# rhymes-ai/Aria

Hardware: NVIDIA H100
Metric: Aria-25.3B bf16 prefill tokens/sec (higher is better)
Workload: dtype bf16

## Files before the change

aria_b200/_lib.py:

```python
from __future__ import annotations

import ctypes as C
import os

_HERE = os.path.dirname(os.path.abspath(__file__))
LIB_PATH = os.environ.get("ARIA_B200_LIB") or os.path.join(_HERE, "libaria_b200.so")

ARIA_OK = 0
B_NK, B_GKN, B_GNK = 0, 1, 2
EPI_LINEAR, EPI_SWIGLU, EPI_HEADS = 0, 1, 2
ACT_NONE, ACT_GELU_TANH, ACT_GELU_NEW = 0, 1, 2

_ERR = {-1: "bad argument", -2: "unsupported shape", -3: "CUDA error"}

vp = C.c_void_p
i32 = C.c_int32
i64 = C.c_int64
f32 = C.c_float


class GemmDesc(C.Structure):

    _fields_ = [
        ("a", vp), ("lda", i64), ("m", i64), ("n", i64), ("k", i64),
        ("b", vp * 3), ("n_seg", i32), ("b_layout", i32),
        ("num_groups", i32), ("group_offsets", vp), ("group_mod", i32),
        ("epilogue", i32), ("act", i32),
        ("bias", vp * 3), ("residual", vp), ("ldr", i64),
        ("out", vp * 3), ("ldo", i64),
        ("head_dim", i32), ("head_ld", i32), ("rows_per_batch", i32), ("pos0", i32),
        ("stride_b", i64), ("stride_h", i64),
        ("rope_mask", i32), ("rope_cos", vp), ("rope_sin", vp), ("position_ids", vp),
        ("group_counts", vp), ("a_rows", i64), ("out_group_base", vp), ("out_group_row0", vp),
    ]


SIGNATURES = {
    "aria_abi_version": (i32, []),
    "aria_build_arch": (C.c_char_p, []),
    "aria_gemm": (i32, [C.POINTER(GemmDesc), vp]),
    "aria_grouped_gemm": (i32, [vp, vp, vp, vp, i64, i64, i64, i32, vp]),
    "aria_offsets_from_counts": (i32, [vp, vp, i32, vp]),
    "aria_router_topk": (i32, [vp, vp, vp, vp, vp, vp, i64, i32, i32, i32, vp]),
    "aria_route_from_logits": (i32, [vp, vp, vp, vp, i64, i32, i32, vp]),
    "aria_route_given_indices": (i32, [vp, vp, vp, vp, i64, i32, i32, vp]),
    "aria_build_permutation": (i32, [vp, vp, vp, vp, vp, i64, i32, i32, i32, vp]),
    "aria_quantize_fp8_cols": (i32, [vp, vp, vp, i32, i64, i64, vp]),
    "aria_grouped_gemm_fp8": (i32, [vp, vp, vp, vp, vp, i64, i64, i64, i32, i32, vp]),
    "aria_permute_quantize_fp8_rows": (i32, [vp, vp, vp, vp, i64, i32, vp]),
    "aria_grouped_gemm_w8a8": (i32, [vp, vp, vp, vp, vp, vp, i64, i64, i64, i32, i32, vp]),
    "aria_grouped_wgrad": (i32, [vp, i64, vp, i64, vp, vp, i64, i64, i64, i32, i32, vp]),
    "aria_moe_block_fwd_workspace_bytes": (i64, [i64, i32, i32, i32, i32, i32]),
    "aria_moe_block_fwd": (i32, [vp, vp, vp, vp, vp, vp, vp, vp, i64, i32, i32, i32, i32, i32, vp, vp, i64, vp, vp]),
    "aria_moe_block_fwd_fp8": (i32, [vp, vp, vp, vp, vp, vp, vp, vp, vp, vp, i64, i32, i32, i32, i32, i32, vp, vp, i64, vp, vp]),
    "aria_moe_block_fwd_w8a8": (i32, [vp, vp, vp, vp, vp, vp, vp, vp, vp, vp, i64, i32, i32, i32, i32, i32, vp, vp, i64, vp, vp]),
    "aria_swiglu_fwd": (i32, [vp, vp, i64, i32, vp]),
    "aria_swiglu_bwd": (i32, [vp, vp, vp, i64, i32, vp]),
    "aria_combine_bwd": (i32, [vp, vp, vp, vp, vp, vp, i64, i32, i32, vp]),
    "aria_router_bwd": (i32, [vp, vp, vp, vp, i64, i32, i32, vp]),
    "aria_router_aux_workspace_bytes": (C.c_size_t, [i32]),
    "aria_router_aux_loss": (i32, [vp, vp, vp, i64, i32, i32, f32, f32, vp, C.c_size_t, vp]),
    "aria_router_aux_bwd": (i32, [vp, vp, vp, i64, i32, i32, f32, f32, f32, vp]),
    "aria_permute_rows": (i32, [vp, vp, vp, i64, i32, vp]),
# ... 65 lines not shown
```

aria_b200/csrc/gemm.cu:

```cuda
#include <cuda_fp8.h>

#include "gemm_common.cuh"

namespace aria {

constexpr int GEMM_STAGES = 4;
constexpr int FP8_LAND_STAGES = 3;
constexpr int FP8_CONVERT_WARPS = 3;
constexpr int PAIR_MIN_ROWS = 2048;
template <int BN, bool B_FP8 = false>
constexpr int gemm_smem_bytes() {
  return 1024  + GEMM_STAGES * (A_STAGE_BYTES + BN * BK * 2) + BM * acc_ld(BN) * 4 + 256  +
         (B_FP8 ? FP8_LAND_STAGES * BN * BK : 0);
}
static_assert(gemm_smem_bytes<128, true>() <= 232448, "fp8 landing ring must fit the opt-in shared memory of a block");

ARIA_DEVICE void e4m3x16_to_bf16(const uint4 v, uint4& lo, uint4& hi) {
  const uint32_t w[4] = {v.x, v.y, v.z, v.w};
  uint32_t o[8];
#pragma unroll
  for (int i = 0; i < 4; ++i) {
#pragma unroll
    for (int h = 0; h < 2; ++h) {
      const __half2_raw hr = __nv_cvt_fp8x2_to_halfraw2(static_cast<__nv_fp8x2_storage_t>(w[i] >> (16 * h)), __NV_E4M3);
      const float2 f = __half22float2(__half2(hr));
      o[2 * i + h] = pack_bf16(f.x, f.y);
    }
  }
  lo = make_uint4(o[0], o[1], o[2], o[3]);
  hi = make_uint4(o[4], o[5], o[6], o[7]);
}

template <bool PAIR> ARIA_DEVICE int first_tile() { return PAIR ? blockIdx.x >> 1 : blockIdx.x; }
template <bool PAIR> ARIA_DEVICE int tile_step() { return PAIR ? gridDim.x >> 1 : gridDim.x; }
template <bool PAIR> ARIA_DEVICE int pair_sched_n(int n_tiles) { return PAIR ? (n_tiles + 1) / 2 : n_tiles; }

template <int BN, bool B_MN>
ARIA_DEVICE void wgmma_tile_k16(float (&acc)[BN / 2], uint64_t da, uint64_t db) {
  if constexpr (BN == 128) wgmma_m64n128_ss<0, B_MN ? 1 : 0>(acc, da, db, 1u);
  else wgmma_m64n144_ss<0, B_MN ? 1 : 0>(acc, da, db, 1u);
}

template <int BN, bool B_MN, int EPI, bool B_FP8 = false, bool PAIR = false>
__global__ void __launch_bounds__(GEMM_THREADS, 1)
gemm_kernel(const __grid_constant__ CUtensorMap tmA, const __grid_constant__ CUtensorMap tmB0,
            const __grid_constant__ CUtensorMap tmB1, const __grid_constant__ CUtensorMap tmB2, const GemmParams p) {
  constexpr int B_STAGE_BYTES = BN * BK * 2;
  constexpr int STAGE_BYTES = A_STAGE_BYTES + B_STAGE_BYTES;
  constexpr int STAGES = GEMM_STAGES;
  constexpr int ACC_LD = acc_ld(BN);
  constexpr int OUT_BN = (EPI == ARIA_EPI_SWIGLU) ? BN / 2 : BN;
  static_assert(BN == 128 || BN == 144, "tile widths with a wgmma wrapper");
  static_assert(!B_FP8 || (B_MN && BN == 128 && EPI != ARIA_EPI_HEADS), "fp8 B: grouped [G, K, N] weights, 128-wide tiles");
  static_assert(!PAIR || (!B_MN && !B_FP8), "CTA pairs: dense K-major bf16 B");
  constexpr int LAND_BYTES = BN * BK;

  uint8_t* smem = smem_1024();
  float* stg = reinterpret_cast<float*>(smem + STAGES * STAGE_BYTES);
  const BarrierRing<STAGES> bar(stg + BM * ACC_LD);
  const BarrierRing<FP8_LAND_STAGES> land_bar(bar.empty + STAGES);
  uint8_t* land = reinterpret_cast<uint8_t*>(bar.full) + 256;

  const int warp = threadIdx.x >> 5;
  const int lane = threadIdx.x & 31;
  const int wg = threadIdx.x >> 7;

  if (warp == 0 && lane == 0) {
    prefetch_tmap(&tmA);
    prefetch_tmap(&tmB0);
    if (p.n_seg > 1 || EPI == ARIA_EPI_SWIGLU) prefetch_tmap(&tmB1);
    if (p.n_seg > 2) prefetch_tmap(&tmB2);
    bar.init(B_FP8 ? 1 + FP8_CONVERT_WARPS : 1, PAIR ? 2 * CONSUMER_WARPS : CONSUMER_WARPS);
    if constexpr (B_FP8) land_bar.init(1, FP8_CONVERT_WARPS);
    fence_mbar_init();
  }
// ... 324 lines not shown
  d.a = a;
  d.lda = k;
  d.m = rows;
  d.n = n;
  d.k = k;
  d.b[0] = b;
  d.n_seg = 1;
  d.b_layout = ARIA_B_GKN;
  d.num_groups = groups;
  d.group_offsets = offsets;
  d.epilogue = epilogue;
  d.out[0] = out;
  d.ldo = n;
  return d;
}

static int64_t max_tiles(const aria_gemm_desc_t* d, int BN, int64_t groups) {
  const bool swiglu = d->epilogue == ARIA_EPI_SWIGLU;
  const int out_bn = swiglu ? BN / 2 : BN;
  const int64_t n_out_total = d->n * (swiglu ? 1 : d->n_seg);
  return (n_out_total + out_bn - 1) / out_bn * ((d->m + BM - 1) / BM + groups);
}

static int gemm_run(const aria_gemm_desc_t* d, const float* b_scale, cudaStream_t stream) {
  ARIA_CHECK_ARG(d != nullptr);
  ARIA_CHECK_ARG(d->a && d->b[0] && d->out[0]);
  ARIA_CHECK_ARG(d->m >= 0 && d->n > 0 && d->k > 0);
  ARIA_CHECK_ARG(d->n % 8 == 0 && d->k % 8 == 0 && d->lda % 8 == 0);
  ARIA_CHECK_ARG(d->n_seg >= 1 && d->n_seg <= 3);
  ARIA_CHECK_ARG(d->num_groups >= 1 && (d->group_mod >= 0 || d->num_groups % (-d->group_mod) == 0));
  ARIA_CHECK_ARG((reinterpret_cast<uintptr_t>(d->a) & 15) == 0 && (reinterpret_cast<uintptr_t>(d->out[0]) & 15) == 0);
  if (d->m == 0) return ARIA_OK;
  const bool b_mn = d->b_layout == ARIA_B_GKN;
  const bool b_gnk = d->b_layout == ARIA_B_GNK;
  const bool swiglu = d->epilogue == ARIA_EPI_SWIGLU;
  if (b_mn) {
    ARIA_CHECK_ARG(d->n_seg == 1);
    ARIA_CHECK_ARG(d->k % BK == 0 || (d->num_groups == 1 && d->group_mod == 0));
    ARIA_CHECK_ARG(d->n % 64 == 0);
    ARIA_CHECK_ARG(d->epilogue != ARIA_EPI_HEADS);
  } else {
    ARIA_CHECK_ARG(d->num_groups == 1 || d->n_seg == 1);
    if (swiglu) ARIA_CHECK_ARG(d->n_seg == 2 && d->b[1]);
    if (b_gnk) ARIA_CHECK_ARG(d->n_seg == 1 && !swiglu && d->epilogue == ARIA_EPI_LINEAR && d->n % 128 == 0);
    else ARIA_CHECK_ARG(d->num_groups == 1);
  }
  if (d->num_groups > 1) ARIA_CHECK_ARG(d->group_offsets != nullptr);
  if (d->group_counts) ARIA_CHECK_ARG(d->group_offsets != nullptr);
  if (d->out_group_base) ARIA_CHECK_ARG(d->out_group_row0 != nullptr && d->epilogue == ARIA_EPI_LINEAR && d->group_offsets != nullptr);
  ARIA_CHECK_ARG(d->a_rows == 0 || d->a_rows >= d->m);

  int BN = 128;
  if (d->epilogue == ARIA_EPI_HEADS) {
    ARIA_CHECK_ARG(d->head_dim > 0 && d->head_dim % 8 == 0 && d->head_ld >= d->head_dim && d->n % d->head_dim == 0);
    if (d->rope_mask) ARIA_CHECK_ARG(d->head_dim == 128 && d->rope_cos && d->rope_sin);
    if (d->n % 128 != 0) {
      ARIA_CHECK_ARG(!d->rope_mask && d->n % 144 == 0);
      BN = 144;
    }
    for (int s = 0; s < d->n_seg; ++s) ARIA_CHECK_ARG(d->out[s] && d->b[s]);
  } else {
    if (swiglu) ARIA_CHECK_ARG(d->n % 64 == 0);
    if (d->n_seg > 1 && !swiglu) ARIA_CHECK_ARG(d->n % BN == 0);
  }

  const bool pair = !b_scale && d->b_layout == ARIA_B_NK && d->num_groups == 1 && !d->group_offsets &&
                    d->epilogue == ARIA_EPI_LINEAR && d->m >= PAIR_MIN_ROWS;

  CUtensorMap tmA, tmB[3];
  int rc = make_tmap_2d(&tmA, d->a, d->k, d->a_rows > 0 ? d->a_rows : d->m, d->lda * 2, BK, pair ? BM / 2 : BM);
  if (rc) return rc;
  if (b_mn) {
    const uint64_t ncols = swiglu ? 2 * d->n : d->n;
    const uint64_t n_weights = d->group_mod > 0 ? d->group_mod : (d->group_mod < 0 ? d->num_groups / (-d->group_mod) : d->num_groups);
    rc = b_scale ? make_tmap_2d(&tmB[0], d->b[0], ncols, n_weights * d->k, ncols, 64, BK, CU_TENSOR_MAP_SWIZZLE_NONE,
                                CU_TENSOR_MAP_DATA_TYPE_UINT8)
                 : make_tmap_2d(&tmB[0], d->b[0], ncols, n_weights * d->k, ncols * 2, 64, BK);
    if (rc) return rc;
    tmB[1] = tmB[0];
    tmB[2] = tmB[0];
  } else {
    const int nb = swiglu ? 2 : d->n_seg;
    const uint32_t box_rows = swiglu ? BN / 2 : BN;
    for (int s = 0; s < 3; ++s) {
      const void* ptr = s < nb ? d->b[s] : d->b[0];
      const uint64_t b_rows = b_gnk ? static_cast<uint64_t>(d->group_mod > 0 ? d->group_mod : (d->group_mod < 0 ? d->num_groups / (-d->group_mod) : d->num_groups)) * d->n : d->n;
      rc = make_tmap_2d(&tmB[s], ptr, d->k, b_rows, d->k * 2, BK, box_rows);
      if (rc) return rc;
    }
  }

  const GemmParams p = gemm_params(d, b_scale);
  const int64_t tiles = max_tiles(d, BN, d->num_groups > 1 ? d->num_groups : 0);
  if (pair) {
    const int64_t m_tiles = (d->m + BM - 1) / BM, pairs = (tiles / m_tiles + 1) / 2 * m_tiles;
    return launch_persistent_pairs<gemm_kernel<128, false, ARIA_EPI_LINEAR, false, true>>(
        "gemm_kernel", GEMM_THREADS, gemm_smem_bytes<128>(), pairs, stream, tmA, tmB[0], tmB[1], tmB[2], p);
  }
#define ARIA_LAUNCH(BN_, MN_, EPI_, ...)                                                                                     \
  return launch_persistent<gemm_kernel<BN_, MN_, EPI_, ##__VA_ARGS__>>("gemm_kernel", GEMM_THREADS,                          \
                                                                       gemm_smem_bytes<BN_, ##__VA_ARGS__>(), tiles, stream, \
                                                                       tmA, tmB[0], tmB[1], tmB[2], p)
  if (b_scale) {
    if (swiglu) ARIA_LAUNCH(128, true, ARIA_EPI_SWIGLU, true);
    ARIA_LAUNCH(128, true, ARIA_EPI_LINEAR, true);
  }
  if (d->epilogue == ARIA_EPI_HEADS) {
    if (BN == 128) ARIA_LAUNCH(128, false, ARIA_EPI_HEADS);
    ARIA_LAUNCH(144, false, ARIA_EPI_HEADS);
  }
  if (swiglu) {
    if (b_mn) ARIA_LAUNCH(128, true, ARIA_EPI_SWIGLU);
    ARIA_LAUNCH(128, false, ARIA_EPI_SWIGLU);
  }
  if (b_mn) ARIA_LAUNCH(128, true, ARIA_EPI_LINEAR);
  ARIA_LAUNCH(128, false, ARIA_EPI_LINEAR);
#undef ARIA_LAUNCH
}

extern "C" int aria_gemm(const aria_gemm_desc_t* d, aria_stream_t stream) {
  return gemm_run(d, nullptr, reinterpret_cast<cudaStream_t>(stream));
}

int aria::grouped_gemm(const void* a, const void* b, const float* b_scale, void* out, const int32_t* offsets, int64_t rows,
                       int64_t k, int64_t n, int32_t groups, int32_t epilogue, cudaStream_t stream) {
  const aria_gemm_desc_t d = grouped_desc(a, b, out, offsets, rows, k, n, groups, epilogue);
  return gemm_run(&d, b_scale, stream);
}

extern "C" int aria_grouped_gemm(const void* a, const void* b, void* out, const int32_t* group_offsets, int64_t rows,
                                 int64_t k, int64_t n, int32_t num_groups, aria_stream_t stream) {
  return grouped_gemm(a, b, nullptr, out, group_offsets, rows, k, n, num_groups, ARIA_EPI_LINEAR,
                      reinterpret_cast<cudaStream_t>(stream));
}

extern "C" int aria_grouped_gemm_fp8(const void* a, const void* b_fp8, const float* b_scale, void* out,
                                     const int32_t* group_offsets, int64_t rows, int64_t k, int64_t n, int32_t num_groups,
                                     int32_t epilogue, aria_stream_t stream) {
  ARIA_CHECK_ARG(a && b_fp8 && b_scale && out && group_offsets);
  ARIA_CHECK_ARG(rows >= 0 && k > 0 && n > 0 && k % BK == 0 && n % 64 == 0 && num_groups >= 1);
  ARIA_CHECK_ARG(epilogue == ARIA_EPI_LINEAR || epilogue == ARIA_EPI_SWIGLU);
  ARIA_CHECK_ARG((reinterpret_cast<uintptr_t>(a) & 15) == 0 && (reinterpret_cast<uintptr_t>(b_fp8) & 15) == 0 &&
                 (reinterpret_cast<uintptr_t>(b_scale) & 15) == 0 && (reinterpret_cast<uintptr_t>(out) & 15) == 0);
  return grouped_gemm(a, b_fp8, b_scale, out, group_offsets, rows, k, n, num_groups, epilogue,
// ... 38 lines not shown
```

aria_b200/csrc/gemm_common.cuh:

```cuda
#pragma once
#include "common.cuh"
#include "ptx.cuh"

namespace aria {

constexpr int BM = 128;
constexpr int BK = 64;
constexpr int A_STAGE_BYTES = BM * BK * 2;
constexpr int GEMM_THREADS = 384;
constexpr int CONSUMER_WARPS = 8;
constexpr int acc_ld(int BN) { return BN + 4; }

struct GemmParams {
  int M, N, K;
  int num_groups;
  const int32_t* group_offsets;
  const int32_t* group_counts;
  const uint64_t* out_group_base;
  const int32_t* out_group_row0;
  int b_group_rows;
  int group_mod;
  int n_seg;
  int act;
  const __nv_bfloat16* bias[3];
  const __nv_bfloat16* residual;
  int64_t ldr;
  __nv_bfloat16* out[3];
  int64_t ldo;
  int head_dim, head_ld, rows_per_batch, pos0;
  int64_t stride_b, stride_h;
  int rope_mask;
  const __nv_bfloat16* rope_cos;
  const __nv_bfloat16* rope_sin;
  const int32_t* position_ids;
// ... 119 lines not shown
    float t = bf16r(0.044715f * p3);
    t = bf16r(x + t);
    t = bf16r(0.7978845608028654f * t);
    t = bf16r(fast_tanh(t));
    t = bf16r(1.0f + t);
    float h = bf16r(0.5f * x);
    return h * t;
  }
  return x;
}

ARIA_DEVICE void ld_acc32(const float* src, uint32_t (&r)[32]) {
#pragma unroll
  for (int i = 0; i < 8; ++i) {
    const uint4 v = *reinterpret_cast<const uint4*>(src + 4 * i);
    r[4 * i] = v.x;
    r[4 * i + 1] = v.y;
    r[4 * i + 2] = v.z;
    r[4 * i + 3] = v.w;
  }
}

template <int BN, int EPI>
ARIA_DEVICE void epilogue_tile(const GemmParams& p, const float* acc, const int n_out_total, const int n_idx,
                               const int64_t grow, const bool row_ok, const int half, const int grp = 0, const int r_in_grp = 0) {
  constexpr int OUT_BN = (EPI == ARIA_EPI_SWIGLU) ? BN / 2 : BN;
  if constexpr (EPI == ARIA_EPI_SWIGLU) {
    __nv_bfloat16* orow = p.out[0] + grow * p.ldo + n_idx * OUT_BN;
    constexpr int NCH = OUT_BN / 32;
    const int cb = (half * NCH / 2) * 32, ce = half ? OUT_BN : (NCH / 2) * 32;
#pragma unroll 1
    for (int c = cb; c < ce; c += 32) {
      uint32_t g[32], u[32];
      ld_acc32(acc + c, g);
      ld_acc32(acc + OUT_BN + c, u);
      uint32_t o[16];
#pragma unroll
      for (int j = 0; j < 32; j += 2) {
        float g0 = __uint_as_float(g[j]), g1 = __uint_as_float(g[j + 1]);
        float u0 = __uint_as_float(u[j]), u1 = __uint_as_float(u[j + 1]);
        bf16r2(g0, g1);
        bf16r2(u0, u1);
        float s0 = fast_silu(g0), s1 = fast_silu(g1);
        bf16r2(s0, s1);
        o[j >> 1] = pack_bf16(s0 * u0, s1 * u1);
      }
      if (row_ok) {
#pragma unroll
        for (int q = 0; q < 4; ++q) {
          const int col = n_idx * OUT_BN + c + q * 8;
          if (col + 8 <= p.N)
            *reinterpret_cast<uint4*>(orow + c + q * 8) = make_uint4(o[q * 4], o[q * 4 + 1], o[q * 4 + 2], o[q * 4 + 3]);
        }
      }
    }
  } else if constexpr (EPI == ARIA_EPI_LINEAR) {
    const int col0 = n_idx * BN;
    const int seg = col0 / p.N;
    const __nv_bfloat16* bias = p.bias[seg];
    __nv_bfloat16* orow = p.out[0] + grow * p.ldo + col0;
    if (p.out_group_base)
      orow = reinterpret_cast<__nv_bfloat16*>(p.out_group_base[grp]) + static_cast<int64_t>(p.out_group_row0[grp] + r_in_grp) * p.ldo + col0;
    const __nv_bfloat16* rrow = (p.residual && row_ok) ? p.residual + grow * p.ldr + col0 : nullptr;
    constexpr int NCH = BN / 32, NCHH = NCH - NCH / 2;
    const int cb = half ? (NCH / 2) * 32 : 0;
    const int n_my = half ? NCH - NCH / 2 : NCH / 2;
    if (n_my == 0) return;
    uint32_t v[2][32];
    uint4 bv[2][4], rv[2][4];
    auto issue = [&](int c, int set) {
      ld_acc32(acc + c, v[set]);
#pragma unroll
      for (int q = 0; q < 4; ++q) {
        const int col = col0 + c + q * 8;
        const bool ok = col + 8 <= n_out_total;
        bv[set][q] = (bias && ok) ? __ldg(reinterpret_cast<const uint4*>(bias + (col - seg * p.N))) : make_uint4(0, 0, 0, 0);
        rv[set][q] = (rrow && ok) ? *reinterpret_cast<const uint4*>(rrow + c + q * 8) : make_uint4(0, 0, 0, 0);
      }
    };
    issue(cb, 0);
// ... 19 lines not shown
          }
        }
#pragma unroll
        for (int j = 0; j < 8; ++j) x[j] = bf16r(x[j]);
        if (p.act != ARIA_ACT_NONE) {
#pragma unroll
          for (int j = 0; j < 8; ++j) x[j] = bf16r(act_apply(x[j], p.act));
        }
        if (row_ok) {
          if (rrow) {
            const uint32_t rw[4] = {rv[set][q].x, rv[set][q].y, rv[set][q].z, rv[set][q].w};
#pragma unroll
            for (int j = 0; j < 4; ++j) {
              x[2 * j] += bf16_lo(rw[j]);
              x[2 * j + 1] += bf16_hi(rw[j]);
            }
          }
          *reinterpret_cast<uint4*>(orow + c + q * 8) =
              make_uint4(pack_bf16(x[0], x[1]), pack_bf16(x[2], x[3]), pack_bf16(x[4], x[5]), pack_bf16(x[6], x[7]));
        }
      }
    }
  } else {
    const int col0 = n_idx * BN;
    const int seg = col0 / p.N;
    const int cseg0 = col0 - seg * p.N;
    const int b = static_cast<int>(grow / p.rows_per_batch);
    const int tok = static_cast<int>(grow - static_cast<int64_t>(b) * p.rows_per_batch);
    __nv_bfloat16* obase = p.out[seg] + b * p.stride_b + static_cast<int64_t>(p.pos0 + tok) * p.head_ld;
    const int pos = row_ok ? (p.position_ids ? p.position_ids[grow] : p.pos0 + tok) : 0;
    const __nv_bfloat16* cs = p.rope_cos + static_cast<int64_t>(pos) * p.head_dim;
    const __nv_bfloat16* sn = p.rope_sin + static_cast<int64_t>(pos) * p.head_dim;
    constexpr int NHC = BN / 64;
#pragma unroll 1
    for (int hc = half * NHC / 2; hc < (half ? NHC : NHC / 2); hc += 1) {
      const int hh = hc >> 1, c = (hc & 1) * 32;
      __nv_bfloat16* orow = obase + (cseg0 / p.head_dim + hh) * p.stride_h;
      const float* th = acc + hh * 128;
      uint32_t lo[32], hi[32];
      ld_acc32(th + c, lo);
      ld_acc32(th + 64 + c, hi);
      uint4 tc_lo[4], ts_lo[4], tc_hi[4], ts_hi[4];
#pragma unroll
      for (int q = 0; q < 4; ++q) {
        tc_lo[q] = __ldg(reinterpret_cast<const uint4*>(cs + c + q * 8));
        ts_lo[q] = __ldg(reinterpret_cast<const uint4*>(sn + c + q * 8));
        tc_hi[q] = __ldg(reinterpret_cast<const uint4*>(cs + 64 + c + q * 8));
// ... 12 lines not shown
            float xh = __uint_as_float(hi[q * 8 + j]);
            bf16r2(xl, xh);
            float cosl = (j & 1) ? bf16_hi(cl[j >> 1]) : bf16_lo(cl[j >> 1]);
            float sinl = (j & 1) ? bf16_hi(sl[j >> 1]) : bf16_lo(sl[j >> 1]);
            float cosh_ = (j & 1) ? bf16_hi(ch[j >> 1]) : bf16_lo(ch[j >> 1]);
            float sinh_ = (j & 1) ? bf16_hi(sh[j >> 1]) : bf16_lo(sh[j >> 1]);
            float a0 = xl * cosl, a1 = -xh * sinl, b0 = xh * cosh_, b1 = xl * sinh_;
            bf16r2(a0, a1);
            bf16r2(b0, b1);
            ol[j] = a0 + a1;
            oh[j] = b0 + b1;
          }
          *reinterpret_cast<uint4*>(orow + c + q * 8) =
              make_uint4(pack_bf16(ol[0], ol[1]), pack_bf16(ol[2], ol[3]), pack_bf16(ol[4], ol[5]), pack_bf16(ol[6], ol[7]));
          *reinterpret_cast<uint4*>(orow + 64 + c + q * 8) =
              make_uint4(pack_bf16(oh[0], oh[1]), pack_bf16(oh[2], oh[3]), pack_bf16(oh[4], oh[5]), pack_bf16(oh[6], oh[7]));
        }
      }
    }
  }
}

template <int BN>
ARIA_DEVICE void heads_store_tile(const GemmParams& p, const float* stg, int cw, int m_idx, int n_idx, int row0, int rows) {
  constexpr int ACC_LD = acc_ld(BN), CH = BN / 8;
  const int col0 = n_idx * BN;
  const int seg = col0 / p.N;
  const int cseg0 = col0 - seg * p.N;
  const __nv_bfloat16* bias = p.bias[seg];
  __nv_bfloat16* out = p.out[seg];
#pragma unroll 1
  for (int i = threadIdx.x & 127; i < 64 * CH; i += 128) {
    const int r = cw * 64 + i / CH, c = (i % CH) * 8;
    const int r_in_grp = m_idx * BM + r;
    const int cs = cseg0 + c;
    if (r_in_grp >= rows || cs + 8 > p.N) continue;
    const float4 lo = *reinterpret_cast<const float4*>(stg + r * ACC_LD + c);
    const float4 hi = *reinterpret_cast<const float4*>(stg + r * ACC_LD + c + 4);
    float x[8] = {lo.x, lo.y, lo.z, lo.w, hi.x, hi.y, hi.z, hi.w};
    if (bias) {
      const uint4 bv = __ldg(reinterpret_cast<const uint4*>(bias + cs));
      const uint32_t bw[4] = {bv.x, bv.y, bv.z, bv.w};
#pragma unroll
      for (int j = 0; j < 4; ++j) {
        x[2 * j] += bf16_lo(bw[j]);
        x[2 * j + 1] += bf16_hi(bw[j]);
      }
    }
    const int grow = row0 + r_in_grp;
    const int b = grow / p.rows_per_batch, tok = grow - b * p.rows_per_batch;
    const int head = cs / p.head_dim, d = cs - head * p.head_dim;
    *reinterpret_cast<uint4*>(out + b * p.stride_b + static_cast<int64_t>(p.pos0 + tok) * p.head_ld + head * p.stride_h + d) =
        make_uint4(pack_bf16(x[0], x[1]), pack_bf16(x[2], x[3]), pack_bf16(x[4], x[5]), pack_bf16(x[6], x[7]));
  }
}

enum class AccScale { NONE, COL, ROW_COL };

template <int BN, int EPI, AccScale SCALE>
ARIA_DEVICE void stage_and_epilogue(const GemmParams& p, float* stg, const ConsumerThread& ct, const float (&acc)[BN / 2],
                                    const float2 (&bsc)[BN / 8], float as0, float as1, int n_out_total, int grp, int m_idx,
                                    int n_idx, int row0, int rows) {
  constexpr int ACC_LD = acc_ld(BN);
  auto scaled = [](float a, float as, float bs) {
    if constexpr (SCALE == AccScale::ROW_COL) return a * as * bs;
    else if constexpr (SCALE == AccScale::COL) return a * bs;
    else return a;
  };
  named_bar_sync(1 + ct.cw, 128);
#pragma unroll
  for (int j = 0; j < BN / 8; ++j) {
    float* d0 = stg + ct.frag_row * ACC_LD + 8 * j + ct.frag_col;
    *reinterpret_cast<float2*>(d0) = make_float2(scaled(acc[4 * j], as0, bsc[j].x), scaled(acc[4 * j + 1], as0, bsc[j].y));
    *reinterpret_cast<float2*>(d0 + 8 * ACC_LD) =
        make_float2(scaled(acc[4 * j + 2], as1, bsc[j].x), scaled(acc[4 * j + 3], as1, bsc[j].y));
  }
  named_bar_sync(1 + ct.cw, 128);
  if constexpr (EPI == ARIA_EPI_HEADS) {
    if (!((p.rope_mask >> (n_idx * BN / p.N)) & 1)) {
      heads_store_tile<BN>(p, stg, ct.cw, m_idx, n_idx, row0, rows);
      return;
    }
  }
  const int r_in_grp = m_idx * BM + ct.epi_row;
  const bool row_ok = r_in_grp < rows;
  const int64_t grow = static_cast<int64_t>(row0) + r_in_grp;
  epilogue_tile<BN, EPI>(p, stg + ct.epi_row * ACC_LD, n_out_total, n_idx, grow, row_ok, ct.half, grp, r_in_grp);
}

}
```

aria_b200/csrc/ptx.cuh:

```cuda
#pragma once
#include <cuda.h>
#include <cuda_bf16.h>
#include <cuda_runtime.h>
#include <stdint.h>

namespace aria {

#define ARIA_DEVICE __device__ __forceinline__

ARIA_DEVICE uint32_t smem_u32(const void* p) { return static_cast<uint32_t>(__cvta_generic_to_shared(p)); }

ARIA_DEVICE uint32_t elect_one() {
  uint32_t pred = 0;
  asm volatile(
      "{\n\t.reg .pred P;\n\t"
      "elect.sync _|P, 0xffffffff;\n\t"
      "selp.b32 %0, 1, 0, P;\n\t}\n"
      : "=r"(pred));
  return pred;
}

ARIA_DEVICE void mbar_init(uint64_t* bar, uint32_t count) {
  asm volatile("mbarrier.init.shared::cta.b64 [%0], %1;" ::"r"(smem_u32(bar)), "r"(count));
}
// ... 120 lines not shown
ARIA_DEVICE void wgmma_m64n128_ss(float (&d)[64], uint64_t da, uint64_t db, uint32_t scale_d) {
  asm volatile(
      "{\n\t.reg .pred p;\n\tsetp.ne.b32 p, %66, 0;\n\t"
      "wgmma.mma_async.sync.aligned.m64n128k16.f32.bf16.bf16 {%0, %1, %2, %3, %4, %5, %6, %7, %8, %9, %10, %11, %12, %13, %14, %15, %16, %17, %18, %19, %20, %21, %22, %23, %24, %25, %26, %27, %28, %29, %30, %31, %32, %33, %34, %35, %36, %37, %38, %39, %40, %41, %42, %43, %44, %45, %46, %47, %48, %49, %50, %51, %52, %53, %54, %55, %56, %57, %58, %59, %60, %61, %62, %63}, %64, %65, p, 1, 1, %67, %68;\n\t}\n"
      : "+f"(d[0]), "+f"(d[1]), "+f"(d[2]), "+f"(d[3]), "+f"(d[4]), "+f"(d[5]), "+f"(d[6]), "+f"(d[7]), "+f"(d[8]), "+f"(d[9]), "+f"(d[10]), "+f"(d[11]), "+f"(d[12]), "+f"(d[13]), "+f"(d[14]), "+f"(d[15]), "+f"(d[16]), "+f"(d[17]), "+f"(d[18]), "+f"(d[19]), "+f"(d[20]), "+f"(d[21]), "+f"(d[22]), "+f"(d[23]), "+f"(d[24]), "+f"(d[25]), "+f"(d[26]), "+f"(d[27]), "+f"(d[28]), "+f"(d[29]), "+f"(d[30]), "+f"(d[31]), "+f"(d[32]), "+f"(d[33]), "+f"(d[34]), "+f"(d[35]), "+f"(d[36]), "+f"(d[37]), "+f"(d[38]), "+f"(d[39]), "+f"(d[40]), "+f"(d[41]), "+f"(d[42]), "+f"(d[43]), "+f"(d[44]), "+f"(d[45]), "+f"(d[46]), "+f"(d[47]), "+f"(d[48]), "+f"(d[49]), "+f"(d[50]), "+f"(d[51]), "+f"(d[52]), "+f"(d[53]), "+f"(d[54]), "+f"(d[55]), "+f"(d[56]), "+f"(d[57]), "+f"(d[58]), "+f"(d[59]), "+f"(d[60]), "+f"(d[61]), "+f"(d[62]), "+f"(d[63])
      : "l"(da), "l"(db), "r"(scale_d), "n"(TA), "n"(TB));
}
template <int TA, int TB>
ARIA_DEVICE void wgmma_m64n64_ss(float (&d)[32], uint64_t da, uint64_t db, uint32_t scale_d) {
  asm volatile(
      "{\n\t.reg .pred p;\n\tsetp.ne.b32 p, %34, 0;\n\t"
      "wgmma.mma_async.sync.aligned.m64n64k16.f32.bf16.bf16 {%0, %1, %2, %3, %4, %5, %6, %7, %8, %9, %10, %11, %12, %13, %14, %15, %16, %17, %18, %19, %20, %21, %22, %23, %24, %25, %26, %27, %28, %29, %30, %31}, %32, %33, p, 1, 1, %35, %36;\n\t}\n"
      : "+f"(d[0]), "+f"(d[1]), "+f"(d[2]), "+f"(d[3]), "+f"(d[4]), "+f"(d[5]), "+f"(d[6]), "+f"(d[7]), "+f"(d[8]), "+f"(d[9]), "+f"(d[10]), "+f"(d[11]), "+f"(d[12]), "+f"(d[13]), "+f"(d[14]), "+f"(d[15]), "+f"(d[16]), "+f"(d[17]), "+f"(d[18]), "+f"(d[19]), "+f"(d[20]), "+f"(d[21]), "+f"(d[22]), "+f"(d[23]), "+f"(d[24]), "+f"(d[25]), "+f"(d[26]), "+f"(d[27]), "+f"(d[28]), "+f"(d[29]), "+f"(d[30]), "+f"(d[31])
      : "l"(da), "l"(db), "r"(scale_d), "n"(TA), "n"(TB));
}
template <int TA, int TB>
ARIA_DEVICE void wgmma_m64n144_ss(float (&d)[72], uint64_t da, uint64_t db, uint32_t scale_d) {
  asm volatile(
      "{\n\t.reg .pred p;\n\tsetp.ne.b32 p, %74, 0;\n\t"
      "wgmma.mma_async.sync.aligned.m64n144k16.f32.bf16.bf16 {%0, %1, %2, %3, %4, %5, %6, %7, %8, %9, %10, %11, %12, %13, %14, %15, %16, %17, %18, %19, %20, %21, %22, %23, %24, %25, %26, %27, %28, %29, %30, %31, %32, %33, %34, %35, %36, %37, %38, %39, %40, %41, %42, %43, %44, %45, %46, %47, %48, %49, %50, %51, %52, %53, %54, %55, %56, %57, %58, %59, %60, %61, %62, %63, %64, %65, %66, %67, %68, %69, %70, %71}, %72, %73, p, 1, 1, %75, %76;\n\t}\n"
      : "+f"(d[0]), "+f"(d[1]), "+f"(d[2]), "+f"(d[3]), "+f"(d[4]), "+f"(d[5]), "+f"(d[6]), "+f"(d[7]), "+f"(d[8]), "+f"(d[9]), "+f"(d[10]), "+f"(d[11]), "+f"(d[12]), "+f"(d[13]), "+f"(d[14]), "+f"(d[15]), "+f"(d[16]), "+f"(d[17]), "+f"(d[18]), "+f"(d[19]), "+f"(d[20]), "+f"(d[21]), "+f"(d[22]), "+f"(d[23]), "+f"(d[24]), "+f"(d[25]), "+f"(d[26]), "+f"(d[27]), "+f"(d[28]), "+f"(d[29]), "+f"(d[30]), "+f"(d[31]), "+f"(d[32]), "+f"(d[33]), "+f"(d[34]), "+f"(d[35]), "+f"(d[36]), "+f"(d[37]), "+f"(d[38]), "+f"(d[39]), "+f"(d[40]), "+f"(d[41]), "+f"(d[42]), "+f"(d[43]), "+f"(d[44]), "+f"(d[45]), "+f"(d[46]), "+f"(d[47]), "+f"(d[48]), "+f"(d[49]), "+f"(d[50]), "+f"(d[51]), "+f"(d[52]), "+f"(d[53]), "+f"(d[54]), "+f"(d[55]), "+f"(d[56]), "+f"(d[57]), "+f"(d[58]), "+f"(d[59]), "+f"(d[60]), "+f"(d[61]), "+f"(d[62]), "+f"(d[63]), "+f"(d[64]), "+f"(d[65]), "+f"(d[66]), "+f"(d[67]), "+f"(d[68]), "+f"(d[69]), "+f"(d[70]), "+f"(d[71])
      : "l"(da), "l"(db), "r"(scale_d), "n"(TA), "n"(TB));
}
ARIA_DEVICE void wgmma_m64n128k32_e4m3_ss(float (&d)[64], uint64_t da, uint64_t db, uint32_t scale_d) {
  asm volatile(
      "{\n\t.reg .pred p;\n\tsetp.ne.b32 p, %66, 0;\n\t"
      "wgmma.mma_async.sync.aligned.m64n128k32.f32.e4m3.e4m3 {%0, %1, %2, %3, %4, %5, %6, %7, %8, %9, %10, %11, %12, %13, %14, %15, %16, %17, %18, %19, %20, %21, %22, %23, %24, %25, %26, %27, %28, %29, %30, %31, %32, %33, %34, %35, %36, %37, %38, %39, %40, %41, %42, %43, %44, %45, %46, %47, %48, %49, %50, %51, %52, %53, %54, %55, %56, %57, %58, %59, %60, %61, %62, %63}, %64, %65, p, 1, 1;\n\t}\n"
      : "+f"(d[0]), "+f"(d[1]), "+f"(d[2]), "+f"(d[3]), "+f"(d[4]), "+f"(d[5]), "+f"(d[6]), "+f"(d[7]), "+f"(d[8]), "+f"(d[9]), "+f"(d[10]), "+f"(d[11]), "+f"(d[12]), "+f"(d[13]), "+f"(d[14]), "+f"(d[15]), "+f"(d[16]), "+f"(d[17]), "+f"(d[18]), "+f"(d[19]), "+f"(d[20]), "+f"(d[21]), "+f"(d[22]), "+f"(d[23]), "+f"(d[24]), "+f"(d[25]), "+f"(d[26]), "+f"(d[27]), "+f"(d[28]), "+f"(d[29]), "+f"(d[30]), "+f"(d[31]), "+f"(d[32]), "+f"(d[33]), "+f"(d[34]), "+f"(d[35]), "+f"(d[36]), "+f"(d[37]), "+f"(d[38]), "+f"(d[39]), "+f"(d[40]), "+f"(d[41]), "+f"(d[42]), "+f"(d[43]), "+f"(d[44]), "+f"(d[45]), "+f"(d[46]), "+f"(d[47]), "+f"(d[48]), "+f"(d[49]), "+f"(d[50]), "+f"(d[51]), "+f"(d[52]), "+f"(d[53]), "+f"(d[54]), "+f"(d[55]), "+f"(d[56]), "+f"(d[57]), "+f"(d[58]), "+f"(d[59]), "+f"(d[60]), "+f"(d[61]), "+f"(d[62]), "+f"(d[63])
      : "l"(da), "l"(db), "r"(scale_d));
}
template <int TB>
ARIA_DEVICE void wgmma_m64n128_rs(float (&d)[64], const uint32_t (&a)[4], uint64_t db) {
  asm volatile(
      "{\n\t.reg .pred p;\n\tsetp.ne.b32 p, 1, 0;\n\t"
      "wgmma.mma_async.sync.aligned.m64n128k16.f32.bf16.bf16 {%0, %1, %2, %3, %4, %5, %6, %7, %8, %9, %10, %11, %12, %13, %14, %15, %16, %17, %18, %19, %20, %21, %22, %23, %24, %25, %26, %27, %28, %29, %30, %31, %32, %33, %34, %35, %36, %37, %38, %39, %40, %41, %42, %43, %44, %45, %46, %47, %48, %49, %50, %51, %52, %53, %54, %55, %56, %57, %58, %59, %60, %61, %62, %63}, {%64, %65, %66, %67}, %68, p, 1, 1, %69;\n\t}\n"
      : "+f"(d[0]), "+f"(d[1]), "+f"(d[2]), "+f"(d[3]), "+f"(d[4]), "+f"(d[5]), "+f"(d[6]), "+f"(d[7]), "+f"(d[8]), "+f"(d[9]), "+f"(d[10]), "+f"(d[11]), "+f"(d[12]), "+f"(d[13]), "+f"(d[14]), "+f"(d[15]), "+f"(d[16]), "+f"(d[17]), "+f"(d[18]), "+f"(d[19]), "+f"(d[20]), "+f"(d[21]), "+f"(d[22]), "+f"(d[23]), "+f"(d[24]), "+f"(d[25]), "+f"(d[26]), "+f"(d[27]), "+f"(d[28]), "+f"(d[29]), "+f"(d[30]), "+f"(d[31]), "+f"(d[32]), "+f"(d[33]), "+f"(d[34]), "+f"(d[35]), "+f"(d[36]), "+f"(d[37]), "+f"(d[38]), "+f"(d[39]), "+f"(d[40]), "+f"(d[41]), "+f"(d[42]), "+f"(d[43]), "+f"(d[44]), "+f"(d[45]), "+f"(d[46]), "+f"(d[47]), "+f"(d[48]), "+f"(d[49]), "+f"(d[50]), "+f"(d[51]), "+f"(d[52]), "+f"(d[53]), "+f"(d[54]), "+f"(d[55]), "+f"(d[56]), "+f"(d[57]), "+f"(d[58]), "+f"(d[59]), "+f"(d[60]), "+f"(d[61]), "+f"(d[62]), "+f"(d[63])
      : "r"(a[0]), "r"(a[1]), "r"(a[2]), "r"(a[3]), "l"(db), "n"(TB));
}
template <int TB>
ARIA_DEVICE void wgmma_m64n64_rs(float (&d)[32], const uint32_t (&a)[4], uint64_t db) {
  asm volatile(
      "{\n\t.reg .pred p;\n\tsetp.ne.b32 p, 1, 0;\n\t"
      "wgmma.mma_async.sync.aligned.m64n64k16.f32.bf16.bf16 {%0, %1, %2, %3, %4, %5, %6, %7, %8, %9, %10, %11, %12, %13, %14, %15, %16, %17, %18, %19, %20, %21, %22, %23, %24, %25, %26, %27, %28, %29, %30, %31}, {%32, %33, %34, %35}, %36, p, 1, 1, %37;\n\t}\n"
      : "+f"(d[0]), "+f"(d[1]), "+f"(d[2]), "+f"(d[3]), "+f"(d[4]), "+f"(d[5]), "+f"(d[6]), "+f"(d[7]), "+f"(d[8]), "+f"(d[9]), "+f"(d[10]), "+f"(d[11]), "+f"(d[12]), "+f"(d[13]), "+f"(d[14]), "+f"(d[15]), "+f"(d[16]), "+f"(d[17]), "+f"(d[18]), "+f"(d[19]), "+f"(d[20]), "+f"(d[21]), "+f"(d[22]), "+f"(d[23]), "+f"(d[24]), "+f"(d[25]), "+f"(d[26]), "+f"(d[27]), "+f"(d[28]), "+f"(d[29]), "+f"(d[30]), "+f"(d[31])
      : "r"(a[0]), "r"(a[1]), "r"(a[2]), "r"(a[3]), "l"(db), "n"(TB));
}
// ... 44 lines not shown
```

include/aria_b200.h:

```cpp
#ifndef ARIA_B200_H
#define ARIA_B200_H

#include <stdint.h>

#ifdef __cplusplus
extern "C" {
#endif

typedef struct CUstream_st* aria_stream_t;

#define ARIA_OK 0
#define ARIA_ERR_BAD_ARG (-1)
#define ARIA_ERR_UNSUPPORTED (-2)
#define ARIA_ERR_CUDA (-3)

int aria_abi_version(void);
const char* aria_build_arch(void);

enum { ARIA_B_NK = 0,
       ARIA_B_GKN = 1,
       ARIA_B_GNK = 2   };
enum { ARIA_EPI_LINEAR = 0,
       ARIA_EPI_SWIGLU = 1,
       ARIA_EPI_HEADS = 2    };
// ... 10 lines not shown
  int32_t num_groups;
  const int32_t* group_offsets;
  int32_t group_mod;
  int32_t epilogue;
  int32_t act;
  const void* bias[3];
  const void* residual;
  int64_t ldr;
  void* out[3];
  int64_t ldo;
  int32_t head_dim, head_ld, rows_per_batch, pos0;
  int64_t stride_b, stride_h;
  int32_t rope_mask;
  const void* rope_cos;
  const void* rope_sin;
  const int32_t* position_ids;
  const int32_t* group_counts;
  int64_t a_rows;
  const void* out_group_base;
  const int32_t* out_group_row0;
} aria_gemm_desc_t;

int aria_gemm(const aria_gemm_desc_t* desc, aria_stream_t stream);

int aria_grouped_gemm(const void* a, const void* b, void* out, const int32_t* group_offsets, int64_t rows,
                      int64_t k, int64_t n, int32_t num_groups, aria_stream_t stream);

int aria_quantize_fp8_cols(const void* w, void* q, float* scale, int32_t G, int64_t K, int64_t N, aria_stream_t stream);
int aria_grouped_gemm_fp8(const void* a, const void* b_fp8, const float* b_scale, void* out, const int32_t* group_offsets,
                          int64_t rows, int64_t k, int64_t n, int32_t num_groups, int32_t epilogue, aria_stream_t stream);

int aria_permute_quantize_fp8_rows(const void* x, const int32_t* src_token, void* q, float* scale, int64_t rows, int32_t d,
                                   aria_stream_t stream);
int aria_grouped_gemm_w8a8(const void* a_fp8, const float* a_scale, const void* b_fp8_nk, const float* b_scale, void* out,
                           const int32_t* group_offsets, int64_t rows, int64_t k, int64_t n, int32_t num_groups, int32_t epilogue,
                           aria_stream_t stream);

int aria_grouped_wgrad(const void* a, int64_t lda, const void* b, int64_t ldb, void* out, const int32_t* group_offsets,
                       int64_t rows, int64_t md, int64_t nd, int32_t num_groups, int32_t num_sources, aria_stream_t stream);

int aria_offsets_from_counts(const int64_t* counts, int32_t* offsets, int32_t num_groups, aria_stream_t stream);

int aria_router_topk(const void* x, const void* w_router, void* logits_out, int32_t* top_idx, void* scores,
                     int32_t* counts, int64_t T, int32_t d, int32_t E, int32_t k, aria_stream_t stream);
int aria_route_from_logits(const void* logits, int32_t* top_idx, void* scores, int32_t* counts, int64_t T,
                           int32_t E, int32_t k, aria_stream_t stream);
// ... 120 lines not shown
```

Before: 17750.

## Add 192-wide CTA-pair GEMM tiles chosen by a wave-count heuristic

Adds a 192-column wgmma tile (m64n192k16) for dense LINEAR GEMMs that run as CTA pairs. A host heuristic picks 192 over 128 when the estimated number of persistent rounds, weighted by an assumed per-tile efficiency factor, comes out lower. To fit shared memory, the epilogue now stages the accumulator in 96-column slices in a loop, with column offsets passed explicitly. The wider tile reuses more of each A load and can cut wave-quantization waste, at the cost of more accumulator registers and an extra staging/barrier pass per tile.

Result: faster. 18160 (median of 6 runs) (+2.3%).

```diff
diff --git a/aria_b200/_lib.py b/aria_b200/_lib.py
--- a/aria_b200/_lib.py
+++ b/aria_b200/_lib.py
@@ -39,6 +39,7 @@
     "aria_abi_version": (i32, []),
     "aria_build_arch": (C.c_char_p, []),
     "aria_gemm": (i32, [C.POINTER(GemmDesc), vp]),
+    "aria_gemm_tile_width": (i32, [C.POINTER(GemmDesc)]),
     "aria_grouped_gemm": (i32, [vp, vp, vp, vp, i64, i64, i64, i32, vp]),
     "aria_offsets_from_counts": (i32, [vp, vp, i32, vp]),
     "aria_router_topk": (i32, [vp, vp, vp, vp, vp, vp, i64, i32, i32, i32, vp]),
diff --git a/aria_b200/csrc/gemm.cu b/aria_b200/csrc/gemm.cu
--- a/aria_b200/csrc/gemm.cu
+++ b/aria_b200/csrc/gemm.cu
@@ -10,10 +10,11 @@
 constexpr int PAIR_MIN_ROWS = 2048;
 template <int BN, bool B_FP8 = false>
 constexpr int gemm_smem_bytes() {
-  return 1024  + GEMM_STAGES * (A_STAGE_BYTES + BN * BK * 2) + BM * acc_ld(BN) * 4 + 256  +
-         (B_FP8 ? FP8_LAND_STAGES * BN * BK : 0);
+  return 1024  + GEMM_STAGES * (A_STAGE_BYTES + BN * BK * 2) + BM * acc_ld(stage_cols(BN)) * 4 +
+         256  + (B_FP8 ? FP8_LAND_STAGES * BN * BK : 0);
 }
 static_assert(gemm_smem_bytes<128, true>() <= 232448, "fp8 landing ring must fit the opt-in shared memory of a block");
+static_assert(gemm_smem_bytes<192>() <= 232448, "ring and staging slice must fit the opt-in shared memory of a block");
 
 ARIA_DEVICE void e4m3x16_to_bf16(const uint4 v, uint4& lo, uint4& hi) {
   const uint32_t w[4] = {v.x, v.y, v.z, v.w};
@@ -38,7 +39,8 @@
 template <int BN, bool B_MN>
 ARIA_DEVICE void wgmma_tile_k16(float (&acc)[BN / 2], uint64_t da, uint64_t db) {
   if constexpr (BN == 128) wgmma_m64n128_ss<0, B_MN ? 1 : 0>(acc, da, db, 1u);
-  else wgmma_m64n144_ss<0, B_MN ? 1 : 0>(acc, da, db, 1u);
+  else if constexpr (BN == 144) wgmma_m64n144_ss<0, B_MN ? 1 : 0>(acc, da, db, 1u);
+  else wgmma_m64n192_ss<0, B_MN ? 1 : 0>(acc, da, db, 1u);
 }
 
 template <int BN, bool B_MN, int EPI, bool B_FP8 = false, bool PAIR = false>
@@ -48,9 +50,10 @@
   constexpr int B_STAGE_BYTES = BN * BK * 2;
   constexpr int STAGE_BYTES = A_STAGE_BYTES + B_STAGE_BYTES;
   constexpr int STAGES = GEMM_STAGES;
-  constexpr int ACC_LD = acc_ld(BN);
+  constexpr int ACC_LD = acc_ld(stage_cols(BN));
   constexpr int OUT_BN = (EPI == ARIA_EPI_SWIGLU) ? BN / 2 : BN;
-  static_assert(BN == 128 || BN == 144, "tile widths with a wgmma wrapper");
+  static_assert(BN == 128 || BN == 144 || BN == 192, "tile widths with a wgmma wrapper");
+  static_assert(BN != 192 || (PAIR && EPI == ARIA_EPI_LINEAR), "192-wide tiles: LINEAR CTA pairs");
   static_assert(!B_FP8 || (B_MN && BN == 128 && EPI != ARIA_EPI_HEADS), "fp8 B: grouped [G, K, N] weights, 128-wide tiles");
   static_assert(!PAIR || (!B_MN && !B_FP8), "CTA pairs: dense K-major bf16 B");
   constexpr int LAND_BYTES = BN * BK;
@@ -421,7 +424,7 @@
   return (n_out_total + out_bn - 1) / out_bn * ((d->m + BM - 1) / BM + groups);
 }
 
-static int gemm_run(const aria_gemm_desc_t* d, const float* b_scale, cudaStream_t stream) {
+static int gemm_check(const aria_gemm_desc_t* d, const float* b_scale) {
   ARIA_CHECK_ARG(d != nullptr);
   ARIA_CHECK_ARG(d->a && d->b[0] && d->out[0]);
   ARIA_CHECK_ARG(d->m >= 0 && d->n > 0 && d->k > 0);
@@ -429,7 +432,6 @@
   ARIA_CHECK_ARG(d->n_seg >= 1 && d->n_seg <= 3);
   ARIA_CHECK_ARG(d->num_groups >= 1 && (d->group_mod >= 0 || d->num_groups % (-d->group_mod) == 0));
   ARIA_CHECK_ARG((reinterpret_cast<uintptr_t>(d->a) & 15) == 0 && (reinterpret_cast<uintptr_t>(d->out[0]) & 15) == 0);
-  if (d->m == 0) return ARIA_OK;
   const bool b_mn = d->b_layout == ARIA_B_GKN;
   const bool b_gnk = d->b_layout == ARIA_B_GNK;
   const bool swiglu = d->epilogue == ARIA_EPI_SWIGLU;
@@ -448,24 +450,41 @@
   if (d->group_counts) ARIA_CHECK_ARG(d->group_offsets != nullptr);
   if (d->out_group_base) ARIA_CHECK_ARG(d->out_group_row0 != nullptr && d->epilogue == ARIA_EPI_LINEAR && d->group_offsets != nullptr);
   ARIA_CHECK_ARG(d->a_rows == 0 || d->a_rows >= d->m);
-
-  int BN = 128;
   if (d->epilogue == ARIA_EPI_HEADS) {
     ARIA_CHECK_ARG(d->head_dim > 0 && d->head_dim % 8 == 0 && d->head_ld >= d->head_dim && d->n % d->head_dim == 0);
     if (d->rope_mask) ARIA_CHECK_ARG(d->head_dim == 128 && d->rope_cos && d->rope_sin);
-    if (d->n % 128 != 0) {
-      ARIA_CHECK_ARG(!d->rope_mask && d->n % 144 == 0);
-      BN = 144;
-    }
+    if (d->n % 128 != 0) ARIA_CHECK_ARG(!d->rope_mask && d->n % 144 == 0);
     for (int s = 0; s < d->n_seg; ++s) ARIA_CHECK_ARG(d->out[s] && d->b[s]);
   } else {
     if (swiglu) ARIA_CHECK_ARG(d->n % 64 == 0);
-    if (d->n_seg > 1 && !swiglu) ARIA_CHECK_ARG(d->n % BN == 0);
-  }
-
-  const bool pair = !b_scale && d->b_layout == ARIA_B_NK && d->num_groups == 1 && !d->group_offsets &&
-                    d->epilogue == ARIA_EPI_LINEAR && d->m >= PAIR_MIN_ROWS;
-
+    if (d->n_seg > 1 && !swiglu) ARIA_CHECK_ARG(d->n % 128 == 0);
+  }
+  return ARIA_OK;
+}
+
+static bool gemm_pairs(const aria_gemm_desc_t* d, const float* b_scale) {
+  return !b_scale && d->b_layout == ARIA_B_NK && d->num_groups == 1 && !d->group_offsets && d->epilogue == ARIA_EPI_LINEAR &&
+         d->m >= PAIR_MIN_ROWS;
+}
+
+constexpr double PAIR192_SPEEDUP = 1.05;
+
+static int gemm_tile_width(const aria_gemm_desc_t* d, bool pair) {
+  if (d->epilogue == ARIA_EPI_HEADS && d->n % 128 != 0) return 144;
+  if (!pair || (d->n_seg > 1 && d->n % 192 != 0)) return 128;
+  const int64_t m_tiles = (d->m + BM - 1) / BM, clusters = sm_count() / 2;
+  const int64_t n_out = d->n * d->n_seg;
+  auto rounds = [&](int bn) {
+    const int64_t n_pairs = ((n_out + bn - 1) / bn + 1) / 2;
+    return static_cast<double>((m_tiles * n_pairs + clusters - 1) / clusters);
+  };
+  return rounds(192) * 1.5 / PAIR192_SPEEDUP < rounds(128) ? 192 : 128;
+}
+
+static int gemm_launch(const aria_gemm_desc_t* d, const float* b_scale, int BN, bool pair, cudaStream_t stream) {
+  const bool b_mn = d->b_layout == ARIA_B_GKN;
+  const bool b_gnk = d->b_layout == ARIA_B_GNK;
+  const bool swiglu = d->epilogue == ARIA_EPI_SWIGLU;
   CUtensorMap tmA, tmB[3];
   int rc = make_tmap_2d(&tmA, d->a, d->k, d->a_rows > 0 ? d->a_rows : d->m, d->lda * 2, BK, pair ? BM / 2 : BM);
   if (rc) return rc;
@@ -493,8 +512,12 @@
   const int64_t tiles = max_tiles(d, BN, d->num_groups > 1 ? d->num_groups : 0);
   if (pair) {
     const int64_t m_tiles = (d->m + BM - 1) / BM, pairs = (tiles / m_tiles + 1) / 2 * m_tiles;
-    return launch_persistent_pairs<gemm_kernel<128, false, ARIA_EPI_LINEAR, false, true>>(
-        "gemm_kernel", GEMM_THREADS, gemm_smem_bytes<128>(), pairs, stream, tmA, tmB[0], tmB[1], tmB[2], p);
+#define ARIA_LAUNCH_PAIRS(BN_)                                                                                             \
+  return launch_persistent_pairs<gemm_kernel<BN_, false, ARIA_EPI_LINEAR, false, true>>(                                   \
+      "gemm_kernel", GEMM_THREADS, gemm_smem_bytes<BN_>(), pairs, stream, tmA, tmB[0], tmB[1], tmB[2], p)
+    if (BN == 192) ARIA_LAUNCH_PAIRS(192);
+    ARIA_LAUNCH_PAIRS(128);
+#undef ARIA_LAUNCH_PAIRS
   }
 #define ARIA_LAUNCH(BN_, MN_, EPI_, ...)                                                                                     \
   return launch_persistent<gemm_kernel<BN_, MN_, EPI_, ##__VA_ARGS__>>("gemm_kernel", GEMM_THREADS,                          \
@@ -517,8 +540,21 @@
 #undef ARIA_LAUNCH
 }
 
+static int gemm_run(const aria_gemm_desc_t* d, const float* b_scale, cudaStream_t stream) {
+  const int rc = gemm_check(d, b_scale);
+  if (rc) return rc;
+  if (d->m == 0) return ARIA_OK;
+  const bool pair = gemm_pairs(d, b_scale);
+  return gemm_launch(d, b_scale, gemm_tile_width(d, pair), pair, stream);
+}
+
 extern "C" int aria_gemm(const aria_gemm_desc_t* d, aria_stream_t stream) {
   return gemm_run(d, nullptr, reinterpret_cast<cudaStream_t>(stream));
+}
+
+extern "C" int aria_gemm_tile_width(const aria_gemm_desc_t* d) {
+  const int rc = gemm_check(d, nullptr);
+  return rc ? rc : gemm_tile_width(d, gemm_pairs(d, nullptr));
 }
 
 int aria::grouped_gemm(const void* a, const void* b, const float* b_scale, void* out, const int32_t* offsets, int64_t rows,
diff --git a/aria_b200/csrc/gemm_common.cuh b/aria_b200/csrc/gemm_common.cuh
--- a/aria_b200/csrc/gemm_common.cuh
+++ b/aria_b200/csrc/gemm_common.cuh
@@ -10,6 +10,7 @@
 constexpr int GEMM_THREADS = 384;
 constexpr int CONSUMER_WARPS = 8;
 constexpr int acc_ld(int BN) { return BN + 4; }
+constexpr int stage_cols(int BN) { return BN == 192 ? 96 : BN; }
 
 struct GemmParams {
   int M, N, K;
@@ -175,11 +176,11 @@
 }
 
 template <int BN, int EPI>
-ARIA_DEVICE void epilogue_tile(const GemmParams& p, const float* acc, const int n_out_total, const int n_idx,
+ARIA_DEVICE void epilogue_tile(const GemmParams& p, const float* acc, const int n_out_total, const int col0,
                                const int64_t grow, const bool row_ok, const int half, const int grp = 0, const int r_in_grp = 0) {
   constexpr int OUT_BN = (EPI == ARIA_EPI_SWIGLU) ? BN / 2 : BN;
   if constexpr (EPI == ARIA_EPI_SWIGLU) {
-    __nv_bfloat16* orow = p.out[0] + grow * p.ldo + n_idx * OUT_BN;
+    __nv_bfloat16* orow = p.out[0] + grow * p.ldo + col0;
     constexpr int NCH = OUT_BN / 32;
     const int cb = (half * NCH / 2) * 32, ce = half ? OUT_BN : (NCH / 2) * 32;
 #pragma unroll 1
@@ -201,14 +202,13 @@
       if (row_ok) {
 #pragma unroll
         for (int q = 0; q < 4; ++q) {
-          const int col = n_idx * OUT_BN + c + q * 8;
+          const int col = col0 + c + q * 8;
           if (col + 8 <= p.N)
             *reinterpret_cast<uint4*>(orow + c + q * 8) = make_uint4(o[q * 4], o[q * 4 + 1], o[q * 4 + 2], o[q * 4 + 3]);
         }
       }
     }
   } else if constexpr (EPI == ARIA_EPI_LINEAR) {
-    const int col0 = n_idx * BN;
     const int seg = col0 / p.N;
     const __nv_bfloat16* bias = p.bias[seg];
     __nv_bfloat16* orow = p.out[0] + grow * p.ldo + col0;
@@ -274,7 +274,6 @@
       }
     }
   } else {
-    const int col0 = n_idx * BN;
     const int seg = col0 / p.N;
     const int cseg0 = col0 - seg * p.N;
     const int b = static_cast<int>(grow / p.rows_per_batch);
@@ -333,9 +332,8 @@
 }
 
 template <int BN>
-ARIA_DEVICE void heads_store_tile(const GemmParams& p, const float* stg, int cw, int m_idx, int n_idx, int row0, int rows) {
+ARIA_DEVICE void heads_store_tile(const GemmParams& p, const float* stg, int cw, int m_idx, int col0, int row0, int rows) {
   constexpr int ACC_LD = acc_ld(BN), CH = BN / 8;
-  const int col0 = n_idx * BN;
   const int seg = col0 / p.N;
   const int cseg0 = col0 - seg * p.N;
   const __nv_bfloat16* bias = p.bias[seg];
@@ -372,31 +370,39 @@
 ARIA_DEVICE void stage_and_epilogue(const GemmParams& p, float* stg, const ConsumerThread& ct, const float (&acc)[BN / 2],
                                     const float2 (&bsc)[BN / 8], float as0, float as1, int n_out_total, int grp, int m_idx,
                                     int n_idx, int row0, int rows) {
-  constexpr int ACC_LD = acc_ld(BN);
+  constexpr int SL = stage_cols(BN);
+  constexpr int ACC_LD = acc_ld(SL);
+  constexpr int OUT_BN = (EPI == ARIA_EPI_SWIGLU) ? BN / 2 : BN;
+  static_assert(SL == BN || (EPI == ARIA_EPI_LINEAR && BN % SL == 0 && SL % 32 == 0), "LINEAR slices of whole 32-column chunks");
   auto scaled = [](float a, float as, float bs) {
     if constexpr (SCALE == AccScale::ROW_COL) return a * as * bs;
     else if constexpr (SCALE == AccScale::COL) return a * bs;
     else return a;
   };
-  named_bar_sync(1 + ct.cw, 128);
-#pragma unroll
-  for (int j = 0; j < BN / 8; ++j) {
-    float* d0 = stg + ct.frag_row * ACC_LD + 8 * j + ct.frag_col;
-    *reinterpret_cast<float2*>(d0) = make_float2(scaled(acc[4 * j], as0, bsc[j].x), scaled(acc[4 * j + 1], as0, bsc[j].y));
-    *reinterpret_cast<float2*>(d0 + 8 * ACC_LD) =
-        make_float2(scaled(acc[4 * j + 2], as1, bsc[j].x), scaled(acc[4 * j + 3], as1, bsc[j].y));
-  }
-  named_bar_sync(1 + ct.cw, 128);
-  if constexpr (EPI == ARIA_EPI_HEADS) {
-    if (!((p.rope_mask >> (n_idx * BN / p.N)) & 1)) {
-      heads_store_tile<BN>(p, stg, ct.cw, m_idx, n_idx, row0, rows);
-      return;
-    }
-  }
-  const int r_in_grp = m_idx * BM + ct.epi_row;
-  const bool row_ok = r_in_grp < rows;
-  const int64_t grow = static_cast<int64_t>(row0) + r_in_grp;
-  epilogue_tile<BN, EPI>(p, stg + ct.epi_row * ACC_LD, n_out_total, n_idx, grow, row_ok, ct.half, grp, r_in_grp);
-}
-
-}
+#pragma unroll
+  for (int s = 0; s < BN / SL; ++s) {
+    named_bar_sync(1 + ct.cw, 128);
+#pragma unroll
+    for (int i = 0; i < SL / 8; ++i) {
+      const int j = s * SL / 8 + i;
+      float* d0 = stg + ct.frag_row * ACC_LD + 8 * i + ct.frag_col;
+      *reinterpret_cast<float2*>(d0) = make_float2(scaled(acc[4 * j], as0, bsc[j].x), scaled(acc[4 * j + 1], as0, bsc[j].y));
+      *reinterpret_cast<float2*>(d0 + 8 * ACC_LD) =
+          make_float2(scaled(acc[4 * j + 2], as1, bsc[j].x), scaled(acc[4 * j + 3], as1, bsc[j].y));
+    }
+    named_bar_sync(1 + ct.cw, 128);
+    const int col0 = n_idx * OUT_BN + s * SL;
+    if constexpr (EPI == ARIA_EPI_HEADS) {
+      if (!((p.rope_mask >> (n_idx * BN / p.N)) & 1)) {
+        heads_store_tile<SL>(p, stg, ct.cw, m_idx, col0, row0, rows);
+        continue;
+      }
+    }
+    const int r_in_grp = m_idx * BM + ct.epi_row;
+    const bool row_ok = r_in_grp < rows;
+    const int64_t grow = static_cast<int64_t>(row0) + r_in_grp;
+    epilogue_tile<SL, EPI>(p, stg + ct.epi_row * ACC_LD, n_out_total, col0, grow, row_ok, ct.half, grp, r_in_grp);
+  }
+}
+
+}
diff --git a/aria_b200/csrc/ptx.cuh b/aria_b200/csrc/ptx.cuh
--- a/aria_b200/csrc/ptx.cuh
+++ b/aria_b200/csrc/ptx.cuh
@@ -166,6 +166,14 @@
       : "+f"(d[0]), "+f"(d[1]), "+f"(d[2]), "+f"(d[3]), "+f"(d[4]), "+f"(d[5]), "+f"(d[6]), "+f"(d[7]), "+f"(d[8]), "+f"(d[9]), "+f"(d[10]), "+f"(d[11]), "+f"(d[12]), "+f"(d[13]), "+f"(d[14]), "+f"(d[15]), "+f"(d[16]), "+f"(d[17]), "+f"(d[18]), "+f"(d[19]), "+f"(d[20]), "+f"(d[21]), "+f"(d[22]), "+f"(d[23]), "+f"(d[24]), "+f"(d[25]), "+f"(d[26]), "+f"(d[27]), "+f"(d[28]), "+f"(d[29]), "+f"(d[30]), "+f"(d[31]), "+f"(d[32]), "+f"(d[33]), "+f"(d[34]), "+f"(d[35]), "+f"(d[36]), "+f"(d[37]), "+f"(d[38]), "+f"(d[39]), "+f"(d[40]), "+f"(d[41]), "+f"(d[42]), "+f"(d[43]), "+f"(d[44]), "+f"(d[45]), "+f"(d[46]), "+f"(d[47]), "+f"(d[48]), "+f"(d[49]), "+f"(d[50]), "+f"(d[51]), "+f"(d[52]), "+f"(d[53]), "+f"(d[54]), "+f"(d[55]), "+f"(d[56]), "+f"(d[57]), "+f"(d[58]), "+f"(d[59]), "+f"(d[60]), "+f"(d[61]), "+f"(d[62]), "+f"(d[63]), "+f"(d[64]), "+f"(d[65]), "+f"(d[66]), "+f"(d[67]), "+f"(d[68]), "+f"(d[69]), "+f"(d[70]), "+f"(d[71])
       : "l"(da), "l"(db), "r"(scale_d), "n"(TA), "n"(TB));
 }
+template <int TA, int TB>
+ARIA_DEVICE void wgmma_m64n192_ss(float (&d)[96], uint64_t da, uint64_t db, uint32_t scale_d) {
+  asm volatile(
+      "{\n\t.reg .pred p;\n\tsetp.ne.b32 p, %98, 0;\n\t"
+      "wgmma.mma_async.sync.aligned.m64n192k16.f32.bf16.bf16 {%0, %1, %2, %3, %4, %5, %6, %7, %8, %9, %10, %11, %12, %13, %14, %15, %16, %17, %18, %19, %20, %21, %22, %23, %24, %25, %26, %27, %28, %29, %30, %31, %32, %33, %34, %35, %36, %37, %38, %39, %40, %41, %42, %43, %44, %45, %46, %47, %48, %49, %50, %51, %52, %53, %54, %55, %56, %57, %58, %59, %60, %61, %62, %63, %64, %65, %66, %67, %68, %69, %70, %71, %72, %73, %74, %75, %76, %77, %78, %79, %80, %81, %82, %83, %84, %85, %86, %87, %88, %89, %90, %91, %92, %93, %94, %95}, %96, %97, p, 1, 1, %99, %100;\n\t}\n"
+      : "+f"(d[0]), "+f"(d[1]), "+f"(d[2]), "+f"(d[3]), "+f"(d[4]), "+f"(d[5]), "+f"(d[6]), "+f"(d[7]), "+f"(d[8]), "+f"(d[9]), "+f"(d[10]), "+f"(d[11]), "+f"(d[12]), "+f"(d[13]), "+f"(d[14]), "+f"(d[15]), "+f"(d[16]), "+f"(d[17]), "+f"(d[18]), "+f"(d[19]), "+f"(d[20]), "+f"(d[21]), "+f"(d[22]), "+f"(d[23]), "+f"(d[24]), "+f"(d[25]), "+f"(d[26]), "+f"(d[27]), "+f"(d[28]), "+f"(d[29]), "+f"(d[30]), "+f"(d[31]), "+f"(d[32]), "+f"(d[33]), "+f"(d[34]), "+f"(d[35]), "+f"(d[36]), "+f"(d[37]), "+f"(d[38]), "+f"(d[39]), "+f"(d[40]), "+f"(d[41]), "+f"(d[42]), "+f"(d[43]), "+f"(d[44]), "+f"(d[45]), "+f"(d[46]), "+f"(d[47]), "+f"(d[48]), "+f"(d[49]), "+f"(d[50]), "+f"(d[51]), "+f"(d[52]), "+f"(d[53]), "+f"(d[54]), "+f"(d[55]), "+f"(d[56]), "+f"(d[57]), "+f"(d[58]), "+f"(d[59]), "+f"(d[60]), "+f"(d[61]), "+f"(d[62]), "+f"(d[63]), "+f"(d[64]), "+f"(d[65]), "+f"(d[66]), "+f"(d[67]), "+f"(d[68]), "+f"(d[69]), "+f"(d[70]), "+f"(d[71]), "+f"(d[72]), "+f"(d[73]), "+f"(d[74]), "+f"(d[75]), "+f"(d[76]), "+f"(d[77]), "+f"(d[78]), "+f"(d[79]), "+f"(d[80]), "+f"(d[81]), "+f"(d[82]), "+f"(d[83]), "+f"(d[84]), "+f"(d[85]), "+f"(d[86]), "+f"(d[87]), "+f"(d[88]), "+f"(d[89]), "+f"(d[90]), "+f"(d[91]), "+f"(d[92]), "+f"(d[93]), "+f"(d[94]), "+f"(d[95])
+      : "l"(da), "l"(db), "r"(scale_d), "n"(TA), "n"(TB));
+}
 ARIA_DEVICE void wgmma_m64n128k32_e4m3_ss(float (&d)[64], uint64_t da, uint64_t db, uint32_t scale_d) {
   asm volatile(
       "{\n\t.reg .pred p;\n\tsetp.ne.b32 p, %66, 0;\n\t"
diff --git a/include/aria_b200.h b/include/aria_b200.h
--- a/include/aria_b200.h
+++ b/include/aria_b200.h
@@ -56,6 +56,7 @@
 } aria_gemm_desc_t;
 
 int aria_gemm(const aria_gemm_desc_t* desc, aria_stream_t stream);
+int aria_gemm_tile_width(const aria_gemm_desc_t* desc);
 
 int aria_grouped_gemm(const void* a, const void* b, void* out, const int32_t* group_offsets, int64_t rows,
                       int64_t k, int64_t n, int32_t num_groups, aria_stream_t stream);
```
